# lhaippp/DMHomo

Hardware: AMD Instinct MI355X
Metric: sampled images/sec (128x128, s_step=32) (higher is better)
Workload: dtype f32; 1 GPU; DGM CFG-Unet dim=64 128x128 bs=25/GPU s_step=32 cond_scale=3 (BASELINE configs[1]); global_batch=25, cfg_mode=streams, hip_graph=True, weights=seeded random init

## Files before the change

dmhomo_amd/_lib.py:

```python
import ctypes as C
import os

import torch

_HERE = os.path.dirname(os.path.abspath(__file__))
LIB_PATH = os.environ.get('DMH_LIB_PATH') or os.path.join(_HERE, 'libdmhomo_hip.so')

c_f32p = C.c_void_p
c_i64 = C.c_int64
c_int = C.c_int
c_float = C.c_float


ABI_VERSION = 500


class DmhConv(C.Structure):
    _fields_ = [('struct_size', C.c_uint64)] + \
               [(n, C.c_void_p) for n in ('src0', 'src1', 'wpack', 'bias', 'in_coef', 'res', 'res_coef', 'out',
                                          'stats')] + \
               [(n, C.c_int32) for n in ('B', 'Hin', 'Win', 'C0', 'C1', 'Cout', 'KH', 'KW', 'stride', 'upsample2')] + \
               [('in_bound', C.c_void_p), ('in_bound_n', C.c_int32), ('fin_n', C.c_int32), ('fin_w', C.c_void_p),
                ('fin_b', C.c_void_p), ('fin_out', C.c_void_p), ('pix_stats', C.c_void_p), ('pix_eps', C.c_float),
                ('rows', C.c_void_p)]


class DmhPackJob(C.Structure):
    _fields_ = [('src', C.c_void_p), ('ws', C.c_void_p), ('wpack', C.c_void_p), ('Cout', C.c_int32), ('C0', C.c_int32),
                ('C1', C.c_int32), ('KH', C.c_int32), ('transposed', C.c_int32)]


class DmhStep(C.Structure):
    _fields_ = [('objective', C.c_int32), ('clip', C.c_int32), ('mode', C.c_int32), ('cond_scale', C.c_float),
                ('sqrt_recip_ac', C.c_float), ('sqrt_recipm1_ac', C.c_float), ('sqrt_ac', C.c_float),
                ('sqrt_1m_ac', C.c_float), ('c0', C.c_float), ('c1', C.c_float), ('c2', C.c_float)]


SIGNATURES = {
    'dmh_last_error': (C.c_char_p, []),
    'dmh_version': (c_int, []),
    'dmh_ws_standardize': (c_int, [c_f32p, c_f32p, c_int, c_int, c_float, C.c_void_p]),
    'dmh_conv_pack_floats': (c_i64, [c_int, c_int, c_int, c_int, c_int]),
    'dmh_pack_conv_weight': (c_int, [c_f32p, c_f32p, c_int, c_int, c_int, c_int, c_int, C.c_void_p]),
    'dmh_pack_conv_weights_multi': (c_int, [C.c_void_p, c_int, c_float, C.c_void_p]),
    'dmh_conv_up2_pack_floats': (c_i64, [c_int, c_int]),
    'dmh_pack_conv_weight_up2': (c_int, [c_f32p, c_f32p, c_int, c_int, C.c_void_p]),
    'dmh_conv_tiles': (c_int, [c_int, c_int, c_int, c_int]),
    'dmh_conv2d': (c_int, [C.POINTER(DmhConv), C.c_void_p]),
    'dmh_rows_from_keep': (c_int, [C.c_void_p, c_int, c_int, C.c_void_p, C.c_void_p]),
    'dmh_gn_finalize': (c_int, [c_f32p, c_int, c_f32p, c_f32p, c_f32p, c_i64, c_f32p, c_int, c_int, c_int, c_int,
                                c_float, C.c_void_p, C.c_void_p]),
    'dmh_gn_finalize_bound': (c_int, [c_f32p, c_int, c_f32p, c_f32p, c_f32p, c_i64, c_f32p, c_f32p, c_int, c_int, c_int,
                                      c_int, c_float, C.c_void_p, C.c_void_p]),
    'dmh_gn_silu_residual': (c_int, [c_f32p, c_f32p, c_f32p, c_f32p, c_int, c_int, c_int, C.c_void_p, C.c_void_p]),
    'dmh_gn_silu_residual_stats': (c_int, [c_f32p, c_f32p, c_f32p, c_f32p, c_f32p, c_int, c_int, c_int, c_float, C.c_void_p,
                                           C.c_void_p]),
    'dmh_chan_layernorm': (c_int, [c_f32p, c_f32p, c_f32p, c_f32p, c_i64, c_int, c_float, C.c_void_p, c_i64, C.c_void_p]),
# ... 170 lines not shown
```

dmhomo_amd/csrc/conv.hip:

```cpp
#include <stdlib.h>

#include "common.h"

#include "conv_args.h"
#include "weight_image.h"

template <int KH, int KW, int S, int UPS, int KC, int TH, int TW>
struct ConvCfg {
  static constexpr int BM = TH * TW;
  static constexpr int MB = BM / 128;
  static constexpr int IN_H = (TH - 1) * S + KH;
  static constexpr int IN_W = (TW - 1) * S + KW;
  static constexpr int IN_PIX = IN_H * IN_W;
  static constexpr int KCP = KC + 4;
  static constexpr int C4 = KC / 4;
  static constexpr int NLOAD = (IN_PIX * C4 + 255) / 256;
  static constexpr int WL = 64 * C4 / 256;
  static constexpr int PAD = (S == 1) ? (KH / 2) : (KH == 4 ? 1 : 0);
  static constexpr int IN_FLOATS = IN_PIX * KCP;
  static constexpr int W_FLOATS = 64 * KCP;
  static constexpr int EPI_BYTES = 4 * 32 * 68 * 4;
  static constexpr int MAIN_BYTES = (IN_FLOATS + 2 * W_FLOATS) * 4;
  static constexpr int LDS_BYTES = MAIN_BYTES > EPI_BYTES ? MAIN_BYTES : EPI_BYTES;
};
// ... 314 lines not shown
  DMH_REQUIRE(w && w_out && Cout > 0 && K > 0, "dmh_ws_standardize: bad arguments");
  hipLaunchKernelGGL(ws_standardize_kernel, dim3(Cout), dim3(256), 0, (hipStream_t)stream, w, w_out, K, eps);
  DMH_CHECK_LAUNCH("dmh_ws_standardize");
  return DMH_OK;
}

extern "C" int dmh_conv2d(const DmhConv* d, void* stream) {
  DMH_REQUIRE(d && d->struct_size == sizeof(DmhConv),
              "dmh_conv2d: DmhConv.struct_size is %llu, this library's DmhConv has %llu bytes (header / library mismatch)",
              d ? (unsigned long long)d->struct_size : 0ull, (unsigned long long)sizeof(DmhConv));
  DMH_REQUIRE(d->src0 && d->wpack, "dmh_conv2d: null pointer");
  DMH_REQUIRE(d->B > 0 && d->Hin > 0 && d->Win > 0 && d->C0 > 0 && d->Cout > 0, "dmh_conv2d: bad shape");
  DMH_REQUIRE(d->C0 % 4 == 0 && (!d->src1 || d->C1 % 4 == 0),
              "dmh_conv2d: input channels must be a multiple of 4 (got %d, %d)", d->C0, d->C1);
  DMH_REQUIRE(!(d->in_coef && d->src1), "dmh_conv2d: the GroupNorm prologue applies to a single source");
  DMH_REQUIRE(!(d->res_coef && !d->res), "dmh_conv2d: res_coef without res");
  DMH_REQUIRE(d->Cout % 4 == 0, "dmh_conv2d: Cout must be a multiple of 4 (got %d)", d->Cout);
  DMH_REQUIRE(!d->in_bound || (d->in_coef && d->in_bound_n > 0 && d->in_bound_n <= 64),
              "dmh_conv2d: in_bound needs in_coef and 1..64 bounds per sample (got %d)", d->in_bound_n);
  hipStream_t st = (hipStream_t)stream;
  const int Hout = conv_out_dim(d->Hin, d->KH, d->stride, d->upsample2);
  const int Wout = conv_out_dim(d->Win, d->KW, d->stride, d->upsample2);
  const int key = d->KH * 100 + d->stride * 10 + d->upsample2;
  DMH_REQUIRE(d->KH == d->KW, "dmh_conv2d: non-square kernel");
  if (d->fin_w) {
    DMH_REQUIRE(d->fin_out && d->fin_n > 0 && d->fin_n <= 8, "dmh_conv2d: fin_w needs fin_out and 1 <= fin_n <= 8 (got %d)",
                d->fin_n);
    DMH_REQUIRE(d->KH == 1 && d->stride == 1 && d->Cout <= 64 && use_f16x3(1, 1),
                "dmh_conv2d: the fused final projection rides on the 1x1 fp16-piece kernel with Cout <= 64 (got %dx%d, Cout %d)",
                d->KH, d->KW, d->Cout);
  } else {
    DMH_REQUIRE(d->out, "dmh_conv2d: null pointer");
  }
  DMH_REQUIRE(!d->pix_stats || (d->KH == 1 && d->stride == 1 && d->Cout == 64 && use_f16x3(1, 1)),
              "dmh_conv2d: pix_stats rides on the 1x1 fp16-piece kernel with Cout == 64 (got %dx%d, Cout %d)", d->KH, d->KW,
              d->Cout);
  switch (key) {
    case 110:
      if (use_f16x3(1, 1)) return dmh_f16x3_launch(d, Hout, Wout, st);
      return launch_conv<1, 1, 1, 0, 32, 16, 16>(d, Hout, Wout, st);
    case 310:
      switch (conv3_variant()) {
        case 6: return dmh_wino_launch(d, Hout, Wout, st);
        case 9: return dmh_f16x3_launch(d, Hout, Wout, st);
        default: return launch_conv<3, 3, 1, 0, 32, 16, 16, 2>(d, Hout, Wout, st);
      }
    case 311:
      switch (conv3_variant()) {
        case 6: return dmh_wino_launch(d, Hout, Wout, st);
        case 9: return dmh_f16x3_launch(d, Hout, Wout, st);
        default: return launch_conv<3, 3, 1, 1, 32, 16, 16, 2>(d, Hout, Wout, st);
      }
    case 312:
      DMH_REQUIRE(use_f16x3(3, 1) && !d->src1 && d->Cout % 64 == 0 && !d->stats,
                  "dmh_conv2d: the sub-pixel upsampling conv needs the fp16-piece kernels, one source, Cout %% 64 == 0, no stats");
      return dmh_f16x3_launch_up2(d, Hout, Wout, st);
    case 710:
      if (use_f16x3(7, 1)) return dmh_f16x3_launch(d, Hout, Wout, st);
      return launch_conv<7, 7, 1, 0, 16, 16, 16>(d, Hout, Wout, st);
    case 420:
      if (use_f16x3_s2d(4, 2, d->C0, d->src1 ? d->C1 : 0)) {
        DMH_REQUIRE(!d->in_coef, "dmh_conv2d: the 4x4 / stride-2 conv takes no GroupNorm prologue");
        return dmh_f16x3_launch(d, Hout, Wout, st);
      }
      return launch_conv<4, 4, 2, 0, 16, 8, 16>(d, Hout, Wout, st);
    case 220:
      DMH_REQUIRE(d->Hin % 2 == 0 && d->Win % 2 == 0, "dmh_conv2d: 2x2/s2 needs even input size");
      return launch_conv<2, 2, 2, 0, 16, 8, 16>(d, Hout, Wout, st);
    default:
// ... 5 lines not shown
```

dmhomo_amd/csrc/conv_args.h:

```cpp
#pragma once
#include "common.h"

typedef float floatx16 __attribute__((ext_vector_type(16)));

struct ConvArgs {
  const float* src0;
  const float* src1;
  const float* wpack;
  const float* bias;
  const float* in_coef;
  const float* res;
  const float* res_coef;
  float* out;
  float* stats;
  const float* oscale;
  const float* in_bound;
  int in_bound_n;
  int fin_n;
  const float* fin_w;
  const float* fin_b;
  float* fin_out;
  float* pix_stats;
  float pix_eps;
  int B, Hin, Win, C0, C1, Cout, Hout, Wout;
  int nch0, nch1, tilesX, tilesY;
  int ablate;
  int xcd;
  const int32_t* rows;
};


static inline ConvArgs fill_conv_args(const DmhConv* d, int Hout, int Wout, int KC, int TH, int TW) {
  ConvArgs a;
  a.src0 = d->src0;
  a.src1 = d->src1;
  a.wpack = d->wpack;
  a.bias = d->bias;
  a.in_coef = d->in_coef;
  a.res = d->res;
  a.res_coef = d->res_coef;
  a.out = d->out;
  a.stats = d->stats;
  a.oscale = nullptr;
  a.in_bound = d->in_coef ? d->in_bound : nullptr;
  a.in_bound_n = d->in_bound_n;
  a.fin_n = d->fin_w ? d->fin_n : 0;
  a.fin_w = d->fin_w;
  a.fin_b = d->fin_b;
  a.fin_out = d->fin_out;
  a.pix_stats = d->pix_stats;
  a.pix_eps = d->pix_eps;
  a.B = d->B;
  a.Hin = d->Hin;
  a.Win = d->Win;
  a.C0 = d->C0;
  a.C1 = d->src1 ? d->C1 : 0;
  a.Cout = d->Cout;
  a.Hout = Hout;
  a.Wout = Wout;
  a.nch0 = cdiv(a.C0, KC);
  a.nch1 = cdiv(a.C1, KC);
// ... 134 lines not shown
      if (p.pix_stats) {
#pragma unroll
        for (int i = 0; i < NR; ++i) {
          float s = (val[i].x + val[i].y) + (val[i].z + val[i].w);
          s = lanes_sum<16>(s);
          const float mean = s / 64.0f;
          const float dx_ = val[i].x - mean, dy_ = val[i].y - mean, dz_ = val[i].z - mean, dw_ = val[i].w - mean;
          float qsum = (dx_ * dx_ + dy_ * dy_) + (dz_ * dz_ + dw_ * dw_);
          qsum = lanes_sum<16>(qsum);
          if (c4 == 0 && okr[i]) {
            float* ps = p.pix_stats + (oo[i] / (size_t)p.Cout) * 2;
            ps[0] = mean;
            ps[1] = 1.0f / sqrtf(qsum / 64.0f + p.pix_eps);
          }
        }
      }
    }
#pragma unroll
    for (int i = 0; i < NR; ++i) {
      if (okr[i] && (!FIN || p.out)) st4(p.out + oo[i], val[i]);
      const float k = okr[i] ? 1.f : 0.f;
      const float vx = val[i].x * k, vy = val[i].y * k, vz = val[i].z * k, vw = val[i].w * k;
      s1.x += vx;
      s1.y += vy;
      s1.z += vz;
      s1.w += vw;
      s2.x = fmaf(vx, vx, s2.x);
      s2.y = fmaf(vy, vy, s2.y);
      s2.z = fmaf(vz, vz, s2.z);
      s2.w = fmaf(vw, vw, s2.w);
    }
  }

  template <int WM, int WN, int TH>
  __device__ __forceinline__ void write_stats_grid(const ConvArgs& p, float* lds, int ty, int tx, int by = -1) {
    if (by < 0) by = blockIdx.y;
    if (!p.stats) return;
    const int lane = threadIdx.x & 63, wave = threadIdx.x >> 6, tid = threadIdx.x;
    s1.x = rows_sum(s1.x);
    s1.y = rows_sum(s1.y);
    s1.z = rows_sum(s1.z);
    s1.w = rows_sum(s1.w);
    s2.x = rows_sum(s2.x);
    s2.y = rows_sum(s2.y);
    s2.z = rows_sum(s2.z);
    s2.w = rows_sum(s2.w);
    __syncthreads();
    float* red = lds;
    if (lane < 16) {
      float* q = red + (wave * 64 + c4 * 4) * 2;
      q[0] = s1.x;
      q[1] = s2.x;
      q[2] = s1.y;
      q[3] = s2.y;
      q[4] = s1.z;
      q[5] = s2.z;
      q[6] = s1.w;
      q[7] = s2.w;
    }
    __syncthreads();
    if (tid < 128) {
      const int q = tid >> 6, c = tid & 63;
      const int g = WN == 1 ? q : 0, wnq = WN == 1 ? 0 : q;
      const int chan = (by * WN + wnq) * 64 + c;
      const int srow = ty * (TH / 8) + g;
      if (chan < p.Cout && srow * 8 < p.Hout) {
// ... 51 lines not shown
```

dmhomo_amd/csrc/conv_f16x3.hip:

```cpp
#include <stdlib.h>

#include "common.h"

#include "conv_args.h"
#include "weight_image.h"

typedef _Float16 half8 __attribute__((ext_vector_type(8)));
typedef _Float16 half4 __attribute__((ext_vector_type(4)));
typedef float float4v __attribute__((ext_vector_type(4)));

namespace {

constexpr int KC = 32;
constexpr int PITCH = 160;
constexpr int STEP_U4 = 4 * 64;

template <int KH, int KW, int S, int UPS, int TH, int TW, int WM, int WN>
struct F16Cfg {
  static_assert(WM * WN == 4, "four waves per workgroup");
  static constexpr bool SUB = UPS == 3;
  static_assert(SUB || TH * TW == WM * 64, "64 pixels per wave");
  static_assert(!SUB || (KH == 2 && KW == 2 && S == 1 && TH == 4 && TW == 16 && WM == 4 && WN == 1), "sub-pixel geometry");
  static constexpr int IN_H = SUB ? TH + 2 : (TH - 1) * S + KH;
  static constexpr int IN_W = SUB ? TW + 2 : (TW - 1) * S + KW;
  static constexpr int IN_PIX = IN_H * IN_W;
  static constexpr int QS = UPS == 4 ? 2 : 3, NQ = 1 << QS;
  static constexpr int NLOAD = (IN_PIX * NQ + 255) / 256;
  static constexpr int PAD = UPS == 2 ? 0 : ((S == 1) ? (KH / 2) : (KH == 4 ? 1 : 0));
  static constexpr int ROWP = IN_W * PITCH;
  static constexpr int IN_BYTES = IN_H * ROWP;
  static constexpr int EPI_BYTES = 4 * 32 * EpilogueRows::EP * 4;
  static constexpr int TILE_BYTES = IN_BYTES > EPI_BYTES ? IN_BYTES : EPI_BYTES;
  static constexpr int LDS_BYTES = TILE_BYTES + 16;
};

__device__ __forceinline__ unsigned absbits(float x) { return __float_as_uint(x) & 0x7fffffffu; }

__device__ __forceinline__ int64_t f16x3_frag_floats_dev(int Cout, int C0, int C1, int T) {
  return (int64_t)((Cout + 63) / 64) * ((C0 + KC - 1) / KC + (C1 + KC - 1) / KC) * T * 2 * STEP_U4 * 4;
}

}

template <int KH, int KW, int S, int UPS, int TH, int TW, int WM, int WN>
__global__ __launch_bounds__(256, 2) void conv_f16x3_kernel(ConvArgs p) {
  using Cfg = F16Cfg<KH, KW, S, UPS, TH, TW, WM, WN>;
  constexpr bool PK = UPS == 4;
  constexpr int IN_W = Cfg::IN_W, IN_PIX = Cfg::IN_PIX, NLOAD = Cfg::NLOAD, NTAPS = PK ? (KH * KW + 1) / 2 : KH * KW,
                ROWP = Cfg::ROWP;

  extern __shared__ __attribute__((aligned(16))) float lds[];
  unsigned char* in_tile = reinterpret_cast<unsigned char*>(lds);
  unsigned* mxslot = reinterpret_cast<unsigned*>(in_tile + Cfg::TILE_BYTES);

  const int tid = threadIdx.x;
  const int lane = tid & 63;
  const int wave = tid >> 6;
  const int wave_u = __builtin_amdgcn_readfirstlane(wave);
  const int kg = lane >> 4;
  const int l15 = lane & 15;
  const int wm = wave / WN, wn = wave % WN;

  int t = blockIdx.x, by = blockIdx.y, nb = gridDim.x;
  if (p.rows) {
    nb = p.tilesX * p.tilesY * p.rows[0];
    const int lin = t + by * (int)gridDim.x;
    if (lin >= nb * (int)gridDim.y) return;
    t = lin % nb;
    by = lin / nb;
  }
  if (p.xcd) {
    const int total = nb * gridDim.y, lin = t + by * nb;
    const int q = total >> 3, r = total & 7, xcd = lin & 7, local = lin >> 3;
    const int nl = xcd * q + min(xcd, r) + local;
    if (p.xcd == 2) {
      by = nl % (int)gridDim.y;
      t = nl / (int)gridDim.y;
    } else {
// ... 318 lines not shown
            float4v& c = acc[mb][(st & 1) * 2 + nb];
            const half8 g1 = __builtin_bit_cast(half8, bq[st % NB][nb * 2]), g2 = __builtin_bit_cast(half8, bq[st % NB][nb * 2 + 1]);
            const half8 h1 = DMH_A(mb, 0), h2 = DMH_A(mb, 1);
            asm("v_mfma_f32_16x16x32_f16 %0, %1, %4, %0\n\t"
                "v_mfma_f32_16x16x32_f16 %0, %2, %3, %0\n\t"
                "v_mfma_f32_16x16x32_f16 %0, %1, %3, %0"
                : "+v"(c) : "v"(g1), "v"(g2), "v"(h1), "v"(h2));
          }
#undef DMH_A
      }
    }
#pragma unroll
    for (int mb = 0; mb < 4; mb += 2)
      asm volatile("s_nop 15" : "+v"(acc[mb][0]), "+v"(acc[mb][1]), "+v"(acc[mb][2]), "+v"(acc[mb][3]), "+v"(acc[mb + 1][0]),
                   "+v"(acc[mb + 1][1]), "+v"(acc[mb + 1][2]), "+v"(acc[mb + 1][3]));
    __builtin_amdgcn_sched_barrier(0);
    STAMP(4)
  }

#ifdef DMH_STAMPS
  if (!(p.ablate & 4))
#endif
  {
    constexpr int EP = EpilogueRows::EP;
    const float inv_s = __uint_as_float((unsigned)(e_run - 14) << 23);
    float* wl = lds + wave * (32 * EP);
    EpilogueRows er(p, b, n0);
    if (UPS == 3 && p.oscale) er.osc = ld4(p.oscale + nt * 64 + er.c4 * 4);
    er.osc.x *= inv_s;
    er.osc.y *= inv_s;
    er.osc.z *= inv_s;
    er.osc.w *= inv_s;
    __syncthreads();
#pragma unroll
    for (int hb = 0; hb < 2; ++hb) {
#pragma unroll
      for (int m2 = 0; m2 < 2; ++m2)
#pragma unroll
        for (int nb = 0; nb < 4; ++nb)
          *reinterpret_cast<float4v*>(wl + (m2 * 16 + l15) * EP + nb * 16 + kg * 4) = acc[hb * 2 + m2][nb];
      __builtin_amdgcn_fence(__ATOMIC_RELEASE, "wavefront");
      __builtin_amdgcn_wave_barrier();
      __builtin_amdgcn_fence(__ATOMIC_ACQUIRE, "wavefront");
      if (UPS == 3) er.template store_rows<TW>(p, wl, hb * 32, oy0, ox0, 2, wm >> 1, wm & 1);
      else er.template store_rows<TW, (KH == 1 && KW == 1 && WN == 1 && UPS == 0)>(p, wl, wm * 64 + hb * 32, oy0, ox0);
    }
#ifdef DMH_STAMPS
    STAMP(5)
    if (p.stats && lane == 0 && by == 0) {
      const int stiles = ((p.Hout + 7) / 8) * p.tilesX;
      unsigned long long* d = reinterpret_cast<unsigned long long*>(
                                  p.stats + ((size_t)(b * stiles + (ty * (TH / 8)) * p.tilesX + tx) * p.Cout) * 2) + wave * 8;
      for (int i = 0; i < 6; ++i) d[i] = tk[i];
      d[6] = t_now - t_begin;
      d[7] = __builtin_amdgcn_s_memrealtime() - rt_begin;
    }
#else
    er.template write_stats_grid<WM, WN, TH>(p, lds, ty, tx, by);
#endif
  }
}
#undef STAMP

__global__ __launch_bounds__(64) void f16x3_wscale_kernel(const float* __restrict__ w, float* __restrict__ oscale,
                                                           int Cout, int K) {
  const int o = blockIdx.x;
// ... 122 lines not shown
  if (f16x3_pk(C0, C1, KH)) return (int64_t)cdiv(Cout, 64) * 25 * 2 * STEP_U4 * 4;
  return (int64_t)cdiv(Cout, 64) * (cdiv(C0, KC) + cdiv(C1, KC)) * KH * KW * 2 * STEP_U4 * 4;
}

int64_t dmh_f16x3_pack_floats(int Cout, int C0, int C1, int KH, int KW) {
  return f16x3_frag_floats(Cout, C0, C1, KH, KW) + (int64_t)cdiv(Cout, 64) * 64;
}

int dmh_f16x3_pack(const float* w, float* wpack, int Cout, int C0, int C1, int KH, int KW, hipStream_t st) {
  const bool s2d = KH == 4;
  if (!s2d && !f16x3_pk(C0, C1, KH)) {
    const DmhPackJob job = {w, nullptr, wpack, Cout, C0, C1, KH, 0};
    return dmh_f16x3_pack_multi(&job, 1, 0.f, st);
  }
  const int64_t frag = f16x3_frag_floats(Cout, C0, C1, KH, KW);
  float* oscale = wpack + frag;
  hipLaunchKernelGGL(f16x3_wscale_kernel, dim3(cdiv(Cout, 64) * 64), dim3(64), 0, st, w, oscale, Cout, C0 * KH * KW);
  const int64_t total = frag * 2;
  hipLaunchKernelGGL(pack_f16x3_weight_kernel, dim3((unsigned)cdiv64(total, 256)), dim3(256), 0, st, w, oscale,
                     reinterpret_cast<_Float16*>(wpack), Cout, C0, s2d ? 4 : 25, s2d ? 4 * C0 / KC : 1, total, s2d ? 1 : 0);
  DMH_CHECK_LAUNCH("dmh_pack_conv_weight(f16x3)");
  return DMH_OK;
}

template <int KH, int KW, int S, int UPS, int TH, int TW, int WM, int WN>
static int launch_f16x3(const DmhConv* d, int Hout, int Wout, hipStream_t st) {
  using Cfg = F16Cfg<KH, KW, S, UPS, TH, TW, WM, WN>;
  ConvArgs a = fill_conv_args(d, Hout, Wout, KC, TH, TW);
  if (UPS == 2) a.nch0 = 4 * a.C0 / KC;
  a.oscale = d->wpack + f16x3_frag_floats(d->Cout, a.C0, a.C1, UPS == 2 ? 4 : KH, UPS == 2 ? 4 : KW);
#ifdef DMH_STAMPS
  if (const char* e = getenv("DMH_WINO_ABLATE")) a.ablate = atoi(e);
#endif
  auto kern = conv_f16x3_kernel<KH, KW, S, UPS, TH, TW, WM, WN>;
  DMH_RAISE_LDS_ONCE(kern, Cfg::LDS_BYTES, "dmh_conv2d(f16x3)");
  static const int xcd_deep = [] {
    const char* e = getenv("DMH_CONV_XCD_DEEP");
    return e ? atoi(e) : 32;
  }();
  if (xcd_deep > 0 && Hout <= xcd_deep && cdiv(a.Cout, 64 * WN) > 1) a.xcd = 2;
  dim3 grid(a.tilesX * a.tilesY * a.B, cdiv(a.Cout, 64 * WN));
  hipLaunchKernelGGL(kern, grid, dim3(256), Cfg::LDS_BYTES, st, a);
  DMH_CHECK_LAUNCH("dmh_conv2d(f16x3)");
  return DMH_OK;
}

__global__ void subpixel_weight_kernel(const float* __restrict__ w, float* __restrict__ wv, int Cout, int Cin) {
  const int64_t idx = (int64_t)blockIdx.x * blockDim.x + threadIdx.x;
  const int64_t total = (int64_t)4 * Cout * Cin * 4;
  if (idx >= total) return;
  const int tb = idx & 1, ta = (idx >> 1) & 1;
  int64_t r = idx >> 2;
  const int c = r % Cin;
  r /= Cin;
  const int o = r % Cout, par = r / Cout;
  const int dy = par >> 1, dx = par & 1;
  const int ky0 = dy == 0 ? (ta == 0 ? 0 : 1) : (ta == 0 ? 0 : 2), ky1 = dy == 0 ? (ta == 0 ? 0 : 2) : (ta == 0 ? 1 : 2);
  const int kx0 = dx == 0 ? (tb == 0 ? 0 : 1) : (tb == 0 ? 0 : 2), kx1 = dx == 0 ? (tb == 0 ? 0 : 2) : (tb == 0 ? 1 : 2);
  const float* wk = w + ((size_t)o * Cin + c) * 9;
  float s = 0.f;
  for (int ky = ky0; ky <= ky1; ++ky)
    for (int kx = kx0; kx <= kx1; ++kx) s += wk[ky * 3 + kx];
  wv[idx] = s;
}

int64_t dmh_f16x3_up2_pack_floats(int Cout, int C0) {
// ... 47 lines not shown
```

dmhomo_amd/engine.py:

```python
import torch

from . import ops
from .layout import ATTN_SCALE, HIDDEN, sinusoidal_freq, unet_layout

FUSED_FINAL = True


class _Res:
    __slots__ = ('conv1', 'g1', 'b1', 'conv2', 'g2', 'b2', 'res', 'ss_off', 'cout')


class _Attn:
    __slots__ = ('linear', 'ln_g', 'qkv', 'pla', 'plo', 'out', 'out_g')


class UnetEngine:
    def __init__(self, module, groups=8):
        self.module = module
        self.groups = groups
        self._sig = None
        self._rows = None

    def _signature(self):
        return (getattr(self.module, '_dmh_epoch', 0),) + tuple((p.data_ptr(), p._version) for p in self.module.parameters())

    def ensure_prepared(self):
        sig = self._signature()
        if sig != self._sig:
            self.prepare()
            self._sig = sig

    def prepare(self):
        sd = {k: v.detach() for k, v in self.module.named_parameters()}
        dev = next(iter(sd.values())).device
        if dev.type != 'cuda':
            raise RuntimeError('dmhomo_amd: the UNet must live on the GPU (call .cuda()); there is no CPU path')
        f32 = lambda k: sd[k].to(torch.float32).contiguous()
        pb = ops.PackBatch()
# ... 56 lines not shown
        for n in L.nodes:
            k = n.keys
            if n.kind == 'res':
                b = res(n)
            elif n.kind in ('linattn', 'attn'):
                b = attn(n)
            elif n.kind == 'unshuffle':
                w22 = f32(k['w']).reshape(n.cout, n.c0, 2, 2).contiguous()
                b = ops.PackedConv(w22, f32(k['b']), n.c0, 0, stride=2, batch=pb)
            else:
                b = conv(k['w'], k['b'], n.c0, stride=2 if n.kind == 'down4' else 1, ups=1 if n.kind == 'up3' else 0)
            self.blocks.append((n, b))
        pb.run()
        nxt = [b for _, b in self.blocks[1:]] + [None]
        self._pixel_stats = [isinstance(a, _Attn) and a.pla is not None for a in nxt]
        self.final_w = f32('final_conv.weight').reshape(L.out_dim, -1).contiguous()
        self.final_b = f32('final_conv.bias')
        res_nodes = [n for n in L.nodes if n.kind == 'res']
        self.mlp_wt = torch.cat([f32(n.keys['mlp_w']).t() for n in res_nodes], dim=1).contiguous()
        self.mlp_b = torch.cat([f32(n.keys['mlp_b']) for n in res_nodes]).contiguous()

    def _res(self, r, x0, x1, ss_all, pixel_stats=False, pre=None, final=None, keep_out=True, fin_out=None):
        B, H, W, _ = x0.shape
        hw = H * W
        rows = self._rows
        y1, st1 = pre if pre is not None else ops.conv2d(r.conv1, x0, x1, want_stats=True, rows=rows)
        ss = ss_all[:, r.ss_off:r.ss_off + 2 * r.cout]
        coef1, bound1 = ops.gn_finalize(st1, r.g1, r.b1, hw, self.groups, ss, want_bound=True, rows=rows)
        y2, st2 = ops.conv2d(r.conv2, y1, in_coef=coef1, want_stats=True, in_bound=bound1, rows=rows)
        coef2 = ops.gn_finalize(st2, r.g2, r.b2, hw, self.groups, rows=rows)
        if final is not None:
            return ops.conv2d(r.res, x0, x1, res=y2, res_coef=coef2, final=final, keep_out=keep_out, fin_out=fin_out, rows=rows)
        if r.res is not None:
            if pixel_stats and r.cout == 64 and r.res.k == 1 and ops.f16x3_default():
                return ops.conv2d(r.res, x0, x1, res=y2, res_coef=coef2, pixel_stats=True, rows=rows)
            x = ops.conv2d(r.res, x0, x1, res=y2, res_coef=coef2, rows=rows)
            return (x, None) if pixel_stats else x
        assert x1 is None
        if pixel_stats:
            if r.cout in ops.PIXEL_STATS_FUSABLE:
                return ops.gn_silu_residual(y2, coef2, x0, pixel_stats=True, rows=rows)
            return ops.gn_silu_residual(y2, coef2, x0, rows=rows), None
        return ops.gn_silu_residual(y2, coef2, x0, rows=rows)

    def _attn(self, a, x, stats=None):
        rows = self._rows
        if a.plo is not None:
            return ops.linear_attention_fused(x, a.ln_g, a.pla, ATTN_SCALE, out=a.plo, stats=stats, rows=rows)
        if a.pla is not None:
            o = ops.linear_attention_fused(x, a.ln_g, a.pla, ATTN_SCALE, stats=stats, rows=rows)
            y = ops.conv2d(a.out, o, rows=rows)
            return ops.chan_layernorm(y, a.out_g, res=x, rows=rows)
        xn = ops.chan_layernorm(x, a.ln_g, rows=rows)
        qkv = ops.conv2d(a.qkv, xn, rows=rows)
        if a.linear:
            o = ops.linear_attention_core(qkv, ATTN_SCALE, rows=rows)
            y = ops.conv2d(a.out, o, rows=rows)
            return ops.chan_layernorm(y, a.out_g, res=x, rows=rows)
        o = ops.attention_core(qkv, ATTN_SCALE, rows=rows)
        return ops.conv2d(a.out, o, res=x, rows=rows)

    def embed(self, time, class_rows, reps):
        B = time.shape[0]
        td = self.t_w2.shape[1]
        cond = torch.empty((reps * B, self.emb_dim), device=time.device, dtype=torch.float32)
        se = ops.fourier_embed(time, self.fourier_w) if self.fourier_w is not None else ops.sinusoidal_embed(time, self.freq)
        hmid = ops.linear(se, self.t_w1, self.t_b1, act_out='gelu')
        for r in range(reps):
            ops.linear(hmid, self.t_w2, self.t_b2, out=cond[r * B:(r + 1) * B, :td])
        if self.has_classes:
            for r, (classes, keep) in enumerate(class_rows):
                ce = ops.class_embed(classes, keep, self.c_table, self.c_null)
                cm = ops.linear(ce, self.c_w1, self.c_b1, act_out='gelu')
                ops.linear(cm, self.c_w2, self.c_b2, out=cond[r * B:(r + 1) * B, td:])
        return cond

    def ss_tables(self, times):
        self.ensure_prepared()
        assert self.has_classes and self.emb_dim == 2 * self.t_w2.shape[1] and self.emb_dim % 4 == 0
        dev, td = self.mlp_wt.device, self.t_w2.shape[1]
        t = torch.as_tensor(list(times), dtype=torch.int64).to(dev)
        ncls = self.c_table.shape[0]
        cls = torch.arange(ncls + 1, dtype=torch.int64, device=dev).clamp(max=ncls - 1)
# ... 63 lines not shown
```

dmhomo_amd/ops.py:

```python
import ctypes as C

import os

import torch

from . import _lib
from ._lib import call, ptr, lib

F32 = torch.float32


def _empty(shape, like, dtype=F32):
    return torch.empty(shape, device=like.device, dtype=dtype)


def ws_standardize(w, eps=1e-5, out=None):
    w = w.detach().contiguous()
    out = torch.empty_like(w) if out is None else out
    cout = w.shape[0]
    call('dmh_ws_standardize', ptr(w), ptr(out), cout, w.numel() // cout, float(eps))
    return out


class PackBatch:
# ... 59 lines not shown
        if own:
            batch.run()

    def repack(self):
        if self._up2:
            call('dmh_pack_conv_weight_up2', ptr(self._w), ptr(self.wpack), self.cout, self.c0)
        else:
            call('dmh_pack_conv_weight', ptr(self._w), ptr(self.wpack), self.cout, self.c0, self.c1, self.k, self.k)


def conv_out_hw(pc, h, w):
    if pc.upsample2:
        return h * 2, w * 2
    if pc.stride == 2:
        return h // 2, w // 2
    return h, w


CONV_LOG = None


def rows_from_keep(keep, extra=0):
    B = keep.shape[0]
    rows = torch.empty((1 + B + extra,), device=keep.device, dtype=torch.int32)
    call('dmh_rows_from_keep', ptr(keep, torch.uint8), B, int(extra), ptr(rows, torch.int32))
    return rows


def _rows(rows):
    return ptr(rows, torch.int32)


def conv2d(pc, src0, src1=None, in_coef=None, res=None, res_coef=None, want_stats=False, in_bound=None, final=None,
           keep_out=True, pixel_stats=False, eps=1e-5, fin_out=None, rows=None):
    B, H, W, c0 = src0.shape
    assert c0 == pc.c0 and (pc.c1 == 0) == (src1 is None), (src0.shape, pc.c0, pc.c1)
    if src1 is not None:
        assert src1.shape == (B, H, W, pc.c1), (src1.shape, pc.c1)
    ho, wo = conv_out_hw(pc, H, W)
    assert keep_out or final is not None
    out = _empty((B, ho, wo, pc.cout), src0) if keep_out else None
    fin_w = fin_b = None
    if final is not None:
        fin_w, fin_b = final
        assert fin_w.shape[1] == pc.cout and fin_w.is_contiguous() and not want_stats, (fin_w.shape, pc.cout)
        if fin_out is None:
            fin_out = _empty((B, fin_w.shape[0], ho, wo), src0)
        assert fin_out.shape == (B, fin_w.shape[0], ho, wo) and fin_out.is_contiguous() and fin_out.dtype == F32
    else:
        assert fin_out is None
    pst = None
    if pixel_stats:
        assert final is None and not want_stats and pc.cout == 64 and pc.k == 1, (pc.cout, pc.k)
        pst = _empty((B, ho * wo, 2), src0)
    stats = None
    if want_stats:
        tiles = lib().dmh_conv_tiles(ho, wo, pc.k, pc.stride)
        stats = _empty((B, tiles, pc.cout, 2), src0)
    if res is not None:
        assert res.shape == (B, ho, wo, pc.cout), (res.shape, (B, ho, wo, pc.cout))
    d = _lib.DmhConv(C.sizeof(_lib.DmhConv), ptr(src0), ptr(src1), ptr(pc.wpack), ptr(pc.bias), ptr(in_coef), ptr(res), ptr(res_coef),
                     ptr(out), ptr(stats), B, H, W, pc.c0, pc.c1, pc.cout, pc.k, pc.k, pc.stride, pc.upsample2,
                     ptr(in_bound), 0 if in_bound is None else in_bound.shape[1],
                     0 if fin_w is None else fin_w.shape[0], ptr(fin_w), ptr(fin_b), ptr(fin_out), ptr(pst), float(eps), _rows(rows))
    if CONV_LOG is not None:
        e0, e1 = torch.cuda.Event(enable_timing=True), torch.cuda.Event(enable_timing=True)
        e0.record()
        call('dmh_conv2d', C.byref(d))
        e1.record()
        CONV_LOG.append((e0, e1, pc.k, pc.stride, B, ho, wo, pc.c0 + pc.c1, pc.cout, pc.upsample2, in_coef is not None))
    else:
        call('dmh_conv2d', C.byref(d))
    if final is not None:
        return out, fin_out
    if pixel_stats:
        return out, pst
    return (out, stats) if want_stats else out


def _ss_arg(ss, B, Cc):
    if ss is None:
        return None, 0
    assert ss.stride(1) == 1 and ss.shape[0] == B and ss.shape[1] == 2 * Cc
    return C.c_void_p(ss.data_ptr()), ss.stride(0)


def gn_finalize(stats, gamma, beta, hw, groups, ss=None, eps=1e-5, want_bound=False, rows=None):
    B, tiles, Cc, _ = stats.shape
    coef = _empty((B, 2, Cc), stats)
    ss_ptr, ss_stride = _ss_arg(ss, B, Cc)
    if want_bound:
        bound = _empty((B, groups), stats)
        call('dmh_gn_finalize_bound', ptr(stats), tiles, ptr(gamma), ptr(beta), ss_ptr, ss_stride, ptr(coef), ptr(bound),
             B, Cc, groups, hw, float(eps), _rows(rows))
        return coef, bound
    call('dmh_gn_finalize', ptr(stats), tiles, ptr(gamma), ptr(beta), ss_ptr, ss_stride, ptr(coef), B, Cc, groups,
         hw, float(eps), _rows(rows))
# ... 845 lines not shown
```

include/dmhomo_hip.h:

```cpp
#ifndef DMHOMO_HIP_H
#define DMHOMO_HIP_H

#include <stdint.h>

#ifdef __cplusplus
extern "C" {
#endif

#define DMH_OK 0
#define DMH_EINVAL (-1)
#define DMH_ELAUNCH (-2)

const char* dmh_last_error(void);
#define DMH_ABI_VERSION 500
int dmh_version(void);


int dmh_ws_standardize(const float* w, float* w_out, int Cout, int K, float eps, void* stream);

int64_t dmh_conv_pack_floats(int Cout, int C0, int C1, int KH, int KW);

int dmh_pack_conv_weight(const float* w_oihw, float* wpack, int Cout, int C0, int C1, int KH, int KW,
                         void* stream);
typedef struct DmhPackJob {
// ... 4 lines not shown
  int32_t transposed;
} DmhPackJob;
int dmh_pack_conv_weights_multi(const DmhPackJob* jobs, int njobs, float ws_eps, void* stream);

int64_t dmh_conv_up2_pack_floats(int Cout, int C0);
int dmh_pack_conv_weight_up2(const float* w_oihw, float* wpack, int Cout, int C0, void* stream);

int dmh_rows_from_keep(const uint8_t* keep, int B, int extra, int32_t* rows, void* stream);

typedef struct DmhConv {
  uint64_t struct_size;
  const float* src0;
  const float* src1;
  const float* wpack;
  const float* bias;
  const float* in_coef;
  const float* res;
  const float* res_coef;
  float* out;
  float* stats;
  int32_t B, Hin, Win, C0, C1, Cout;
  int32_t KH, KW;
  int32_t stride;
  int32_t upsample2;
  const float* in_bound;
  int32_t in_bound_n;
  int32_t fin_n;
  const float* fin_w;
  const float* fin_b;
  float* fin_out;
  float* pix_stats;
  float pix_eps;
  const int32_t* rows;
} DmhConv;

int dmh_conv_tiles(int Hout, int Wout, int KH, int stride);
int dmh_conv2d(const DmhConv* d, void* stream);


int dmh_gn_finalize(const float* stats, int tiles, const float* gamma, const float* beta, const float* ss,
                    int64_t ss_stride, float* coef, int B, int C, int groups, int hw, float eps, const int32_t* rows,
                    void* stream);

int dmh_gn_finalize_bound(const float* stats, int tiles, const float* gamma, const float* beta, const float* ss,
                          int64_t ss_stride, float* coef, float* bound, int B, int C, int groups, int hw, float eps,
                          const int32_t* rows, void* stream);

int dmh_gn_silu_residual(const float* y, const float* coef, const float* res, float* out, int B, int HW, int C,
                         const int32_t* rows, void* stream);

int dmh_gn_silu_residual_stats(const float* y, const float* coef, const float* res, float* out, float* pstats, int B,
                               int HW, int C, float eps, const int32_t* rows, void* stream);

int dmh_chan_layernorm(const float* x, const float* g, const float* res, float* out, int64_t npix, int C,
                       float eps, const int32_t* rows, int64_t pix_per_row, void* stream);

int dmh_linattn_splits(int n);
int64_t dmh_linattn_partial_floats(int B, int n);
int dmh_linattn_context(const float* qkv, float* partial, int B, int n, const int32_t* rows, void* stream);
int dmh_linattn_merge(const float* partial, float* ctx, int B, int n, const int32_t* rows, void* stream);
int dmh_linattn_apply(const float* qkv, const float* ctx, float* out, int B, int n, float scale, const int32_t* rows,
                      void* stream);

int dmh_pixel_stats(const float* x, float* stats, int64_t npix, int C, float eps, const int32_t* rows, int64_t pix_per_row,
                    void* stream);
int64_t dmh_linattn_fused_pack_floats(int C);
// ... 181 lines not shown
```

Before: 89.09 images/s.

## Fuse per-pixel stats and channel layernorm into 1x1 conv epilogue at 128 channels

Adds a pixel-wide epilogue to the 1x1 fp16-piece conv kernel for Cout==128 that reduces across two waves through LDS. It computes per-pixel mean and rstd, and either writes pixel stats or applies channel layernorm with gain and residual directly. This removes a separate chan_layernorm pass after the attention output projection, and a separate stats pass for 128-channel residual convs, saving a full activation round trip. The cost is extra syncthreads and LDS traffic in the epilogue, plus a new kernel instantiation that may use more registers.

```diff
diff --git a/dmhomo_amd/_lib.py b/dmhomo_amd/_lib.py
--- a/dmhomo_amd/_lib.py
+++ b/dmhomo_amd/_lib.py
@@ -22,7 +22,7 @@
                [(n, C.c_int32) for n in ('B', 'Hin', 'Win', 'C0', 'C1', 'Cout', 'KH', 'KW', 'stride', 'upsample2')] + \
                [('in_bound', C.c_void_p), ('in_bound_n', C.c_int32), ('fin_n', C.c_int32), ('fin_w', C.c_void_p),
                 ('fin_b', C.c_void_p), ('fin_out', C.c_void_p), ('pix_stats', C.c_void_p), ('pix_eps', C.c_float),
-                ('rows', C.c_void_p)]
+                ('rows', C.c_void_p), ('ln_g', C.c_void_p), ('ln_res', C.c_void_p), ('ln_eps', C.c_float)]
 
 
 class DmhPackJob(C.Structure):
diff --git a/dmhomo_amd/csrc/conv.hip b/dmhomo_amd/csrc/conv.hip
--- a/dmhomo_amd/csrc/conv.hip
+++ b/dmhomo_amd/csrc/conv.hip
@@ -370,9 +370,20 @@
   } else {
     DMH_REQUIRE(d->out, "dmh_conv2d: null pointer");
   }
-  DMH_REQUIRE(!d->pix_stats || (d->KH == 1 && d->stride == 1 && d->Cout == 64 && use_f16x3(1, 1)),
-              "dmh_conv2d: pix_stats rides on the 1x1 fp16-piece kernel with Cout == 64 (got %dx%d, Cout %d)", d->KH, d->KW,
+  DMH_REQUIRE(!d->pix_stats || (d->KH == 1 && d->stride == 1 && (d->Cout == 64 || d->Cout == 128) && use_f16x3(1, 1)),
+              "dmh_conv2d: pix_stats rides on the 1x1 fp16-piece kernel with Cout == 64 or 128 (got %dx%d, Cout %d)", d->KH, d->KW,
               d->Cout);
+  DMH_REQUIRE(!d->pix_stats || d->Cout == 64 || (!d->stats && !d->fin_w),
+              "dmh_conv2d: pix_stats at Cout == 128 goes without stats and fin_w");
+  DMH_REQUIRE(!((d->pix_stats && d->Cout == 128) || d->ln_g) || (int64_t)d->Hin * d->Win * 512 < ((int64_t)1 << 32),
+              "dmh_conv2d: the pixel-wide epilogue at Cout == 128 addresses a sample with 32-bit byte offsets (got %d x %d)", d->Hin,
+              d->Win);
+  if (d->ln_g) {
+    DMH_REQUIRE(d->KH == 1 && d->stride == 1 && d->Cout == 128 && use_f16x3(1, 1),
+                "dmh_conv2d: ln_g rides on the 1x1 fp16-piece kernel with Cout == 128 (got %dx%d, Cout %d)", d->KH, d->KW, d->Cout);
+    DMH_REQUIRE(d->ln_res && !d->res && !d->res_coef && !d->stats && !d->fin_w && !d->pix_stats,
+                "dmh_conv2d: ln_g needs ln_res and goes without res, stats, fin_w and pix_stats");
+  }
   switch (key) {
     case 110:
       if (use_f16x3(1, 1)) return dmh_f16x3_launch(d, Hout, Wout, st);
diff --git a/dmhomo_amd/csrc/conv_args.h b/dmhomo_amd/csrc/conv_args.h
--- a/dmhomo_amd/csrc/conv_args.h
+++ b/dmhomo_amd/csrc/conv_args.h
@@ -1,4 +1,6 @@
 #pragma once
+#include <type_traits>
+
 #include "common.h"
 
 typedef float floatx16 __attribute__((ext_vector_type(16)));
@@ -27,6 +29,12 @@
   int ablate;
   int xcd;
   const int32_t* rows;
+};
+
+struct ConvPixArgs : ConvArgs {
+  const float* ln_g;
+  const float* ln_res;
+  float ln_eps;
 };
 
 
@@ -227,6 +235,118 @@
     }
   }
 
+  template <typename T>
+  __device__ __forceinline__ T* pix_at(T* base, int pixel) const {
+    using Byte = std::conditional_t<std::is_const<T>::value, const char, char>;
+    return reinterpret_cast<T*>(reinterpret_cast<Byte*>(base) + ((unsigned)pixel * 512u + (cok ? (unsigned)chn * 4u : 0u)));
+  }
+  template <int TW>
+  __device__ __forceinline__ void pix_rows(const ConvPixArgs& p, float* lds, const float* wl, int hb, int row_base, int oy0,
+                                           int ox0) {
+    const int wave = threadIdx.x >> 6;
+    float* mine = lds + wave * (32 * EP) + 64 + hb * 2;
+    const float* theirs = lds + (wave ^ 1) * (32 * EP) + 64 + hb * 2;
+    const size_t sample = (size_t)b * p.Hout * p.Wout;
+    float* outb = p.out + sample * 128;
+    int pix[8];
+    unsigned okm = 0u;
+#pragma unroll
+    for (int i = 0; i < 8; ++i) {
+      const int row = row_base + i * 4 + rsub;
+      const int oy = oy0 + row / TW, ox = ox0 + row % TW;
+      okm |= ((cok && oy < p.Hout && ox < p.Wout) ? 1u : 0u) << i;
+      pix[i] = min(oy, p.Hout - 1) * p.Wout + min(ox, p.Wout - 1);
+    }
+    const float* resb = p.ln_g ? p.ln_res + sample * 128 : (p.res ? p.res + sample * 128 : nullptr);
+    if (resb) {
+#pragma unroll
+      for (int i = 0; i < 8; ++i) rv[i] = ld4(pix_at(resb, pix[i]));
+    }
+    float4 val[8];
+#pragma unroll
+    for (int i = 0; i < 8; ++i) val[i] = ld4(wl + (i * 4 + rsub) * EP + c4 * 4);
+#pragma unroll
+    for (int i = 0; i < 8; ++i) {
+      val[i].x = fmaf(val[i].x, osc.x, bias.x);
+      val[i].y = fmaf(val[i].y, osc.y, bias.y);
+      val[i].z = fmaf(val[i].z, osc.z, bias.z);
+      val[i].w = fmaf(val[i].w, osc.w, bias.w);
+    }
+    if (p.res && !p.ln_g) {
+      if (p.res_coef) {
+#pragma unroll
+        for (int i = 0; i < 8; ++i) {
+          val[i].x += silu_fast(fmaf(ra.x, rv[i].x, rb.x));
+          val[i].y += silu_fast(fmaf(ra.y, rv[i].y, rb.y));
+          val[i].z += silu_fast(fmaf(ra.z, rv[i].z, rb.z));
+          val[i].w += silu_fast(fmaf(ra.w, rv[i].w, rb.w));
+        }
+      } else {
+#pragma unroll
+        for (int i = 0; i < 8; ++i) {
+          val[i].x += rv[i].x;
+          val[i].y += rv[i].y;
+          val[i].z += rv[i].z;
+          val[i].w += rv[i].w;
+        }
+      }
+    }
+    float mean[8], rstd[8];
+#pragma unroll
+    for (int i = 0; i < 8; ++i) {
+      float s = 0.f;
+      s += (val[i].x + val[i].y) + (val[i].z + val[i].w);
+      s = lanes_sum<16>(s);
+      mean[i] = s;
+      if (c4 == 0) mine[(i * 4 + rsub) * EP] = s;
+    }
+    __syncthreads();
+#pragma unroll
+    for (int i = 0; i < 8; ++i) {
+      const float s = mean[i] + theirs[(i * 4 + rsub) * EP];
+      mean[i] = s / 128.0f;
+    }
+#pragma unroll
+    for (int i = 0; i < 8; ++i) {
+      float qsum = 0.f;
+      const float dx = val[i].x - mean[i], dy = val[i].y - mean[i], dz = val[i].z - mean[i], dw = val[i].w - mean[i];
+      qsum += fmaf(dx, dx, dy * dy) + fmaf(dz, dz, dw * dw);
+      qsum = lanes_sum<16>(qsum);
+      rstd[i] = qsum;
+      if (c4 == 0) mine[(i * 4 + rsub) * EP + 1] = qsum;
+    }
+    __syncthreads();
+#pragma unroll
+    for (int i = 0; i < 8; ++i) {
+      const float qsum = rstd[i] + theirs[(i * 4 + rsub) * EP + 1];
+      rstd[i] = 1.0f / sqrtf(qsum / 128.0f + (p.ln_g ? p.ln_eps : p.pix_eps));
+    }
+    if (p.ln_g) {
+      const float4 gg = cok ? ld4(p.ln_g + chn) : make_float4(0.f, 0.f, 0.f, 0.f);
+#pragma unroll
+      for (int i = 0; i < 8; ++i) {
+        float4 o;
+        o.x = (val[i].x - mean[i]) * rstd[i] * gg.x;
+        o.y = (val[i].y - mean[i]) * rstd[i] * gg.y;
+        o.z = (val[i].z - mean[i]) * rstd[i] * gg.z;
+        o.w = (val[i].w - mean[i]) * rstd[i] * gg.w;
+        o.x += rv[i].x;
+        o.y += rv[i].y;
+        o.z += rv[i].z;
+        o.w += rv[i].w;
+        val[i] = o;
+      }
+    } else if (p.pix_stats && n0 == 0 && c4 == 0) {
+      float* psb = p.pix_stats + sample * 2;
+#pragma unroll
+      for (int i = 0; i < 8; ++i)
+        if ((okm >> i) & 1u) *reinterpret_cast<float2*>(psb + (unsigned)pix[i] * 2u) = make_float2(mean[i], rstd[i]);
+    }
+#pragma unroll
+    for (int i = 0; i < 8; ++i)
+      if ((okm >> i) & 1u) st4(pix_at(outb, pix[i]), val[i]);
+  }
+
   template <int WM, int WN, int TH>
   __device__ __forceinline__ void write_stats_grid(const ConvArgs& p, float* lds, int ty, int tx, int by = -1) {
     if (by < 0) by = blockIdx.y;
diff --git a/dmhomo_amd/csrc/conv_f16x3.hip b/dmhomo_amd/csrc/conv_f16x3.hip
--- a/dmhomo_amd/csrc/conv_f16x3.hip
+++ b/dmhomo_amd/csrc/conv_f16x3.hip
@@ -1,4 +1,6 @@
 #include <stdlib.h>
+
+#include <type_traits>
 
 #include "common.h"
 
@@ -42,8 +44,8 @@
 
 }
 
-template <int KH, int KW, int S, int UPS, int TH, int TW, int WM, int WN>
-__global__ __launch_bounds__(256, 2) void conv_f16x3_kernel(ConvArgs p) {
+template <int KH, int KW, int S, int UPS, int TH, int TW, int WM, int WN, bool PIX = false>
+__global__ __launch_bounds__(256, 2) void conv_f16x3_kernel(std::conditional_t<PIX, ConvPixArgs, ConvArgs> p) {
   using Cfg = F16Cfg<KH, KW, S, UPS, TH, TW, WM, WN>;
   constexpr bool PK = UPS == 4;
   constexpr int IN_W = Cfg::IN_W, IN_PIX = Cfg::IN_PIX, NLOAD = Cfg::NLOAD, NTAPS = PK ? (KH * KW + 1) / 2 : KH * KW,
@@ -428,6 +430,22 @@
     er.osc.z *= inv_s;
     er.osc.w *= inv_s;
     __syncthreads();
+    if constexpr (PIX) {
+      static_assert(!PIX || (KH == 1 && KW == 1 && UPS == 0 && WM == 2 && WN == 2 && TH == 8), "the pixel-wide epilogue's layout");
+#pragma unroll
+      for (int hb = 0; hb < 2; ++hb) {
+#pragma unroll
+        for (int m2 = 0; m2 < 2; ++m2)
+#pragma unroll
+          for (int nb = 0; nb < 4; ++nb)
+            *reinterpret_cast<float4v*>(wl + (m2 * 16 + l15) * EP + nb * 16 + kg * 4) = acc[hb * 2 + m2][nb];
+        __builtin_amdgcn_fence(__ATOMIC_RELEASE, "wavefront");
+        __builtin_amdgcn_wave_barrier();
+        __builtin_amdgcn_fence(__ATOMIC_ACQUIRE, "wavefront");
+        er.template pix_rows<TW>(p, lds, wl, hb, wm * 64 + hb * 32, oy0, ox0);
+      }
+      return;
+    }
 #pragma unroll
     for (int hb = 0; hb < 2; ++hb) {
 #pragma unroll
@@ -616,6 +634,20 @@
 #ifdef DMH_STAMPS
   if (const char* e = getenv("DMH_WINO_ABLATE")) a.ablate = atoi(e);
 #endif
+  if constexpr (KH == 1 && UPS == 0 && WN == 2) {
+    if (d->pix_stats || d->ln_g) {
+      ConvPixArgs ap;
+      static_cast<ConvArgs&>(ap) = a;
+      ap.ln_g = d->ln_g;
+      ap.ln_res = d->ln_res;
+      ap.ln_eps = d->ln_eps;
+      auto pkern = conv_f16x3_kernel<KH, KW, S, UPS, TH, TW, WM, WN, true>;
+      DMH_RAISE_LDS_ONCE(pkern, Cfg::LDS_BYTES, "dmh_conv2d(f16x3 pixel epilogue)");
+      hipLaunchKernelGGL(pkern, dim3(a.tilesX * a.tilesY * a.B, 1), dim3(256), Cfg::LDS_BYTES, st, ap);
+      DMH_CHECK_LAUNCH("dmh_conv2d(f16x3 pixel epilogue)");
+      return DMH_OK;
+    }
+  }
   auto kern = conv_f16x3_kernel<KH, KW, S, UPS, TH, TW, WM, WN>;
   DMH_RAISE_LDS_ONCE(kern, Cfg::LDS_BYTES, "dmh_conv2d(f16x3)");
   static const int xcd_deep = [] {
diff --git a/dmhomo_amd/engine.py b/dmhomo_amd/engine.py
--- a/dmhomo_amd/engine.py
+++ b/dmhomo_amd/engine.py
@@ -4,6 +4,7 @@
 from .layout import ATTN_SCALE, HIDDEN, sinusoidal_freq, unet_layout
 
 FUSED_FINAL = True
+FUSED_C128 = True
 
 
 class _Res:
@@ -126,7 +127,7 @@
         if final is not None:
             return ops.conv2d(r.res, x0, x1, res=y2, res_coef=coef2, final=final, keep_out=keep_out, fin_out=fin_out, rows=rows)
         if r.res is not None:
-            if pixel_stats and r.cout == 64 and r.res.k == 1 and ops.f16x3_default():
+            if pixel_stats and (r.cout == 64 or (r.cout == 128 and FUSED_C128)) and r.res.k == 1 and ops.f16x3_default():
                 return ops.conv2d(r.res, x0, x1, res=y2, res_coef=coef2, pixel_stats=True, rows=rows)
             x = ops.conv2d(r.res, x0, x1, res=y2, res_coef=coef2, rows=rows)
             return (x, None) if pixel_stats else x
@@ -143,6 +144,8 @@
             return ops.linear_attention_fused(x, a.ln_g, a.pla, ATTN_SCALE, out=a.plo, stats=stats, rows=rows)
         if a.pla is not None:
             o = ops.linear_attention_fused(x, a.ln_g, a.pla, ATTN_SCALE, stats=stats, rows=rows)
+            if x.shape[-1] == 128 and FUSED_C128 and ops.f16x3_default():
+                return ops.conv2d(a.out, o, ln=(a.out_g, x), rows=rows)
             y = ops.conv2d(a.out, o, rows=rows)
             return ops.chan_layernorm(y, a.out_g, res=x, rows=rows)
         xn = ops.chan_layernorm(x, a.ln_g, rows=rows)
diff --git a/dmhomo_amd/ops.py b/dmhomo_amd/ops.py
--- a/dmhomo_amd/ops.py
+++ b/dmhomo_amd/ops.py
@@ -115,7 +115,7 @@
 
 
 def conv2d(pc, src0, src1=None, in_coef=None, res=None, res_coef=None, want_stats=False, in_bound=None, final=None,
-           keep_out=True, pixel_stats=False, eps=1e-5, fin_out=None, rows=None):
+           keep_out=True, pixel_stats=False, eps=1e-5, fin_out=None, rows=None, ln=None):
     B, H, W, c0 = src0.shape
     assert c0 == pc.c0 and (pc.c1 == 0) == (src1 is None), (src0.shape, pc.c0, pc.c1)
     if src1 is not None:
@@ -134,8 +134,13 @@
         assert fin_out is None
     pst = None
     if pixel_stats:
-        assert final is None and not want_stats and pc.cout == 64 and pc.k == 1, (pc.cout, pc.k)
+        assert final is None and not want_stats and pc.cout in (64, 128) and pc.k == 1, (pc.cout, pc.k)
         pst = _empty((B, ho * wo, 2), src0)
+    ln_g = ln_res = None
+    if ln is not None:
+        ln_g, ln_res = ln
+        assert final is None and not want_stats and not pixel_stats and res is None and pc.cout == 128 and pc.k == 1, (pc.cout, pc.k)
+        assert ln_g.shape == (pc.cout,) and ln_res.shape == (B, ho, wo, pc.cout), (ln_g.shape, ln_res.shape)
     stats = None
     if want_stats:
         tiles = lib().dmh_conv_tiles(ho, wo, pc.k, pc.stride)
@@ -145,7 +150,8 @@
     d = _lib.DmhConv(C.sizeof(_lib.DmhConv), ptr(src0), ptr(src1), ptr(pc.wpack), ptr(pc.bias), ptr(in_coef), ptr(res), ptr(res_coef),
                      ptr(out), ptr(stats), B, H, W, pc.c0, pc.c1, pc.cout, pc.k, pc.k, pc.stride, pc.upsample2,
                      ptr(in_bound), 0 if in_bound is None else in_bound.shape[1],
-                     0 if fin_w is None else fin_w.shape[0], ptr(fin_w), ptr(fin_b), ptr(fin_out), ptr(pst), float(eps), _rows(rows))
+                     0 if fin_w is None else fin_w.shape[0], ptr(fin_w), ptr(fin_b), ptr(fin_out), ptr(pst), float(eps), _rows(rows),
+                     ptr(ln_g), ptr(ln_res), float(eps))
     if CONV_LOG is not None:
         e0, e1 = torch.cuda.Event(enable_timing=True), torch.cuda.Event(enable_timing=True)
         e0.record()
diff --git a/include/dmhomo_hip.h b/include/dmhomo_hip.h
--- a/include/dmhomo_hip.h
+++ b/include/dmhomo_hip.h
@@ -60,6 +60,9 @@
   float* pix_stats;
   float pix_eps;
   const int32_t* rows;
+  const float* ln_g;
+  const float* ln_res;
+  float ln_eps;
 } DmhConv;
 
 int dmh_conv_tiles(int Hout, int Wout, int KH, int stride);
```

Result: no change. 89.67 images/s (median of 6 runs) (+0.7%).
